# fplll/fplll

Measured on AMD Instinct MI355X. Metric: enum nodes/sec (BKZ-60 SVP enumeration, dim-180 q-ary lattice), higher is better.
Workload: dtype f64; 1 GPU; BASELINE configs[2]: beta=60 blocks kappa=0,1,2 of the 180-dim q-ary lattice, one Enumeration::enumerate call per step, radius min(0.99 r,1.1 GH), FastEvaluator(1); pruning=LinearPruningParams(60,30), counting_rule=fplll (after the bound test), summed in 64 bit

## Files before the change

fplll_amd/build.py:

```python
import os
import subprocess
import sys

HERE = os.path.dirname(os.path.abspath(__file__))
ROOT = os.path.dirname(HERE)
CSRC = os.path.join(HERE, "csrc")
LIBDIR = os.path.join(HERE, "lib")

HIP_SOURCES = ["enum_kernel.hip", "enum_walk.hip", "enum_kernel_cvp.hip", "enum_walk_cvp.hip", "enum_walk4.hip", "enum_kernel_list.hip", "enum_walk_list.hip", "enum_kernel_cvp_list.hip", "enum_walk_cvp_list.hip", "enum_deal.hip", "enum_order.hip", "enum_host.hip", "gso_kernel.hip", "gso_sweep2.hip", "lll_kernel.hip", "lll_kernel_early.hip", "hlll_kernel.hip", "hh_blocked.hip", "hh_rows.hip", "hlll_x.hip", "lll_x.hip", "bkz_kernel.hip", "bkzs_kernel.hip", "bkz_kernel_u.hip", "bkzs_kernel_u.hip", "hlll_kernel_u.hip", "hlll_x_u.hip", "lll_x_u.hip", "gso_host.hip", "lll_gram.hip", "gram_host.hip", "cvp_prepare.hip", "list_vectors.hip", "pruner_volume.hip", "pruner_search.hip", "gso_util_host.hip"]
HIP_HEADERS = ["dev_mem.h", "dev_cache.h", "trace.h", "pruner_tables.h", "pruner_engine.h", "enum_device.h", "enum_order.h", "enum_wave.h", "gso_device.h", "gram_device.h", "gso_wave.h", "gso_sweep2.h", "ftx.h", "lll_wave.h", "lll_stream.h", os.path.join(ROOT, "include", "fplll_hip.h")]
HIPCC_FLAGS = [
    "--offload-arch=gfx950", "-O3", "-std=c++17",
    "-ffp-contract=off",
    "-fPIC", "-Wno-unused-value", "-Wno-inline-asm",
]


PER_FILE_FLAGS = {
    "enum_kernel.hip": ["-mllvm", "-structurizecfg-skip-uniform-regions=1", "-Xclang", "-disable-lifetime-markers"],
    "enum_walk.hip": ["-mllvm", "-structurizecfg-skip-uniform-regions=1", "-Xclang", "-disable-lifetime-markers"],
    "enum_kernel_cvp.hip": ["-mllvm", "-structurizecfg-skip-uniform-regions=1", "-Xclang", "-disable-lifetime-markers"],
    "enum_walk_cvp.hip": ["-mllvm", "-structurizecfg-skip-uniform-regions=1", "-Xclang", "-disable-lifetime-markers"],
    "enum_kernel_list.hip": ["-mllvm", "-structurizecfg-skip-uniform-regions=1", "-Xclang", "-disable-lifetime-markers"],
    "enum_walk_list.hip": ["-mllvm", "-structurizecfg-skip-uniform-regions=1", "-Xclang", "-disable-lifetime-markers"],
    "enum_kernel_cvp_list.hip": ["-mllvm", "-structurizecfg-skip-uniform-regions=1", "-Xclang", "-disable-lifetime-markers"],
    "enum_walk_cvp_list.hip": ["-mllvm", "-structurizecfg-skip-uniform-regions=1", "-Xclang", "-disable-lifetime-markers"],
    "enum_walk4.hip": ["-mllvm", "-structurizecfg-skip-uniform-regions=1", "-Xclang", "-disable-lifetime-markers"],
    "bkzs_kernel.hip": ["-mllvm", "-structurizecfg-skip-uniform-regions=1", "-Xclang", "-disable-lifetime-markers"],
    "bkzs_kernel_u.hip": ["-mllvm", "-structurizecfg-skip-uniform-regions=1", "-Xclang", "-disable-lifetime-markers"],
    "bkz_kernel_u.hip": ["-mllvm", "-structurizecfg-skip-uniform-regions=1"],
    "lll_kernel.hip": ["-mllvm", "-structurizecfg-skip-uniform-regions=1"],
    "lll_kernel_early.hip": ["-mllvm", "-structurizecfg-skip-uniform-regions=1"],
    "lll_gram.hip": ["-mllvm", "-structurizecfg-skip-uniform-regions=1"],
    "bkz_kernel.hip": ["-mllvm", "-structurizecfg-skip-uniform-regions=1"],
    "hlll_kernel.hip": ["-mllvm", "-structurizecfg-skip-uniform-regions=1"],
    "hlll_kernel_u.hip": ["-mllvm", "-structurizecfg-skip-uniform-regions=1"],
    "gso_kernel.hip": ["-mllvm", "-structurizecfg-skip-uniform-regions=1"],
}


EXTRA_DEPS = {"lll_kernel_early.hip": ["lll_kernel.hip"], "enum_kernel_cvp.hip": ["enum_kernel.hip"],
              "enum_walk_cvp.hip": ["enum_walk.hip"], "enum_walk4.hip": ["enum_walk.hip"],
              "enum_kernel_list.hip": ["enum_kernel.hip"], "enum_walk_list.hip": ["enum_walk.hip"],
              "enum_kernel_cvp_list.hip": ["enum_kernel.hip"], "enum_walk_cvp_list.hip": ["enum_walk.hip"], "bkz_kernel_u.hip": ["bkz_kernel.hip"],
              "bkzs_kernel_u.hip": ["bkzs_kernel.hip"], "hlll_kernel_u.hip": ["hlll_kernel.hip"],
              "hlll_x_u.hip": ["hlll_x.hip"], "lll_x_u.hip": ["lll_x.hip"]}


def _newer(target, deps):
    if not os.path.exists(target):
        return True
    t = os.path.getmtime(target)
    return any(os.path.exists(d) and os.path.getmtime(d) > t for d in deps)


def _run(cmd, cwd=None):
    print("[build]", " ".join(cmd), flush=True)
    subprocess.check_call(cmd, cwd=cwd)


def hipcc():
    for c in ("hipcc", "/opt/rocm/bin/hipcc"):
        try:
            subprocess.check_output([c, "--version"], stderr=subprocess.STDOUT)
            return c
        except Exception:
            continue
    raise RuntimeError("hipcc not found")


def build_hip(force=False):
    os.makedirs(LIBDIR, exist_ok=True)
    out = os.path.join(LIBDIR, "libfplll_hip.so")
    srcs = [os.path.join(CSRC, s) for s in HIP_SOURCES if os.path.exists(os.path.join(CSRC, s))]
    hdrs = [h if os.path.isabs(h) else os.path.join(CSRC, h) for h in HIP_HEADERS]
    extra = []
    if os.environ.get("FPHIP_GSO_RING"):
        extra.append("-DFPHIP_GSO_RING=" + os.environ["FPHIP_GSO_RING"])
        force = True
    objdir = os.path.join(LIBDIR, "obj")
    os.makedirs(objdir, exist_ok=True)
    objs = []
    relink = force or not os.path.exists(out)
    jobs = []
    for src in srcs:
        obj = os.path.join(objdir, os.path.basename(src) + ".o")
        objs.append(obj)
        more = [os.path.join(CSRC, x) for x in EXTRA_DEPS.get(os.path.basename(src), [])]
        if force or _newer(obj, [src, os.path.abspath(__file__)] + hdrs + more):
            jobs.append([hipcc()] + HIPCC_FLAGS + extra + PER_FILE_FLAGS.get(os.path.basename(src), []) +
                        ["-c", "-o", obj, src])
            relink = True
    if jobs:
        from concurrent.futures import ThreadPoolExecutor
        with ThreadPoolExecutor(max_workers=max(1, min(len(jobs), os.cpu_count() or 1))) as ex:
# ... 62 lines not shown
```

fplll_amd/csrc/enum_host.hip:

```cpp

#include <hip/hip_runtime.h>

#include <algorithm>
#include <chrono>
#include <cmath>
#include <cstdarg>
#include <cstdio>
#include <cstdlib>
#include <cstring>
#include <vector>

#include "../../include/fplll_hip.h"
#include "dev_mem.h"
#include "trace.h"
#include "enum_device.h"
#include "enum_order.h"


namespace fphip
{
template <bool MU_LDS, bool SUBS, bool DUAL>
__global__ void enum_phase_kernel(DevShared *g, HostCtl *h, TaskBuf in, TaskBuf out, int d,
                                  int Lmax, int stop, unsigned task_lo, unsigned task_hi,
                                  const unsigned *idxlist, int launch_idx, int count_nodes,
                                  unsigned budget, const double *xhi_root, double *gstk, int Tsplit,
                                  unsigned *qh, const unsigned *rcnt, unsigned rcap,
                                  unsigned long long bound_init);
template <int NQT, bool SUBS, bool DUAL>
__global__ void enum_top_kernel(DevShared *g, HostCtl *h, TopBuf in, unsigned n_in, TopBuf out_top,
                                int stop, TaskBuf out, double *xhi_root, int d, double maxdist,
                                int count_nodes, int launch_idx, double *gtop);
__global__ void task_key_kernel(TaskBuf in, unsigned n, int d, unsigned long long *keys,
                                const double *xhi_root, const unsigned *slots);
template <bool MU_LDS, bool DUAL, bool CHAIN>
__global__ void enum_walk_kernel(DevShared *g, HostCtl *h, TaskBuf in, TaskBuf out, int d, int Lmax, unsigned task_lo,
                                 unsigned task_hi, const unsigned *idxlist, int launch_idx, int count_nodes,
                                 unsigned budget, const double *xhi_root, double *gstk, int Tsplit, unsigned *qh,
                                 const unsigned *rcnt, unsigned rcap, unsigned long long bound_init);
template <bool MU_LDS, bool DUAL>
__global__ void enum_walk4_kernel(DevShared *g, HostCtl *h, TaskBuf in, TaskBuf out, int d, int Lmax, unsigned task_lo,
                                  unsigned task_hi, const unsigned *idxlist, int launch_idx, int count_nodes,
                                  unsigned budget, const double *xhi_root, double *gstk, int Tsplit, unsigned *qh,
                                  const unsigned *rcnt, unsigned rcap, unsigned long long bound_init);
template <bool MU_LDS, bool SUBS, bool DUAL>
__global__ void enum_phase_cvp_kernel(DevShared *g, HostCtl *h, TaskBuf in, TaskBuf out, int d, int Lmax, int stop,
                                      unsigned task_lo, unsigned task_hi, const unsigned *idxlist, int launch_idx,
                                      int count_nodes, unsigned budget, const double *xhi_root, double *gstk, int Tsplit,
                                      unsigned *qh, const unsigned *rcnt, unsigned rcap, unsigned long long bound_init);
template <bool MU_LDS, bool DUAL, bool CHAIN>
__global__ void enum_walk_cvp_kernel(DevShared *g, HostCtl *h, TaskBuf in, TaskBuf out, int d, int Lmax, unsigned task_lo,
                                     unsigned task_hi, const unsigned *idxlist, int launch_idx, int count_nodes,
                                     unsigned budget, const double *xhi_root, double *gstk, int Tsplit, unsigned *qh,
                                     const unsigned *rcnt, unsigned rcap, unsigned long long bound_init);
template <bool MU_LDS, bool SUBS, bool DUAL>
__global__ void enum_phase_list_kernel(DevShared *g, HostCtl *h, TaskBuf in, TaskBuf out, int d, int Lmax, int stop,
                                       unsigned task_lo, unsigned task_hi, const unsigned *idxlist, int launch_idx,
                                       int count_nodes, unsigned budget, const double *xhi_root, double *gstk, int Tsplit,
                                       unsigned *qh, const unsigned *rcnt, unsigned rcap, unsigned long long bound_init,
                                       ListBuf lst);
template <bool MU_LDS, bool SUBS, bool DUAL>
__global__ void enum_phase_cvp_list_kernel(DevShared *g, HostCtl *h, TaskBuf in, TaskBuf out, int d, int Lmax, int stop,
                                           unsigned task_lo, unsigned task_hi, const unsigned *idxlist, int launch_idx,
                                           int count_nodes, unsigned budget, const double *xhi_root, double *gstk,
                                           int Tsplit, unsigned *qh, const unsigned *rcnt, unsigned rcap,
                                           unsigned long long bound_init, ListBuf lst);
template <bool MU_LDS, bool DUAL, bool CHAIN>
__global__ void enum_walk_list_kernel(DevShared *g, HostCtl *h, TaskBuf in, TaskBuf out, int d, int Lmax, unsigned task_lo,
                                      unsigned task_hi, const unsigned *idxlist, int launch_idx, int count_nodes,
                                      unsigned budget, const double *xhi_root, double *gstk, int Tsplit, unsigned *qh,
                                      const unsigned *rcnt, unsigned rcap, unsigned long long bound_init, ListBuf lst);
template <bool MU_LDS, bool DUAL, bool CHAIN>
__global__ void enum_walk_cvp_list_kernel(DevShared *g, HostCtl *h, TaskBuf in, TaskBuf out, int d, int Lmax,
                                          unsigned task_lo, unsigned task_hi, const unsigned *idxlist, int launch_idx,
                                          int count_nodes, unsigned budget, const double *xhi_root, double *gstk, int Tsplit,
                                          unsigned *qh, const unsigned *rcnt, unsigned rcap, unsigned long long bound_init,
                                          ListBuf lst);
template <bool DUAL>
__global__ void enum_bfs_cvp_kernel(DevShared *g, double maxdist, QueueMem *qm, TaskBuf f0, TaskBuf f1, TaskBuf fin, int L0,
                                    int nlev, int floor_level, float heavy, int count_nodes, int compact_n, int shard_index,
                                    int shard_count);
template <int NQT, bool SUBS, bool DUAL>
__global__ void enum_top_cvp_kernel(DevShared *g, HostCtl *h, TopBuf in, unsigned n_in, TopBuf out_top, int stop,
                                    TaskBuf out, double *xhi_root, int d, double maxdist, int count_nodes, int launch_idx,
                                    double *gtop);
size_t deal_work_bytes(unsigned n);
unsigned deal_tasks_device(hipStream_t s, const unsigned long long *keys, const double *pd, const unsigned *slot_of,
                           unsigned n, unsigned W, unsigned rank, unsigned *mine, void *work, size_t work_bytes);
size_t order_work_bytes(unsigned n);
int order_tasks_device(hipStream_t s, const DevShared *g, TaskBuf in, unsigned n, int d, const unsigned *slots,
                       unsigned *list, void *work, size_t work_bytes, int num_cus, int *sort_passes);
__global__ void task_pack_kernel(TaskBuf in, unsigned lo, unsigned n, double *rec, const double *xhi_root, int xstr);
__global__ void task_unpack_kernel(TaskBuf out, unsigned lo, unsigned n, const double *rec, double *xhi_root, int xstr,
                                   unsigned root_base);
// ... 939 lines not shown
      else if (dual)
        FPHIP_TOP_LAUNCH(2, false, true);
      else if (subs)
        FPHIP_TOP_LAUNCH(2, true, false);
      else
        FPHIP_TOP_LAUNCH(2, false, false);
#undef FPHIP_TOP_LAUNCH
      HIPCHK(ctx, hipGetLastError());
      HIPCHK(ctx, hipEventRecord(ctx->ev[1], ctx->stream));
      uint64_t nsub = 0;
      int rcw       = wait_serving(ctx, d, cb, subcb, user, &nsub);
      if (rcw != FPHIP_OK)
        return rcw;
      float tms = 0;
      HIPCHK(ctx, hipEventElapsedTime(&tms, ctx->ev[0], ctx->ev[1]));
      top_ms += tms;
      ++launch_idx;
      return FPHIP_OK;
    };
    int rct = top_launch(0, 1u, cut, 1u);
    if (rct != FPHIP_OK)
      return rct;
    if (cut > 64)
    {
      unsigned c1 = 0;
      HIPCHK(ctx, hipMemcpy(&c1, ctx->top[1].count, 4, hipMemcpyDeviceToHost));
      if (c1 > cap2)
      {
        snprintf(ctx->err, sizeof ctx->err, "more than %u top tasks: the block stays on the CPU enumerator", cap2);
        return FPHIP_UNSUPPORTED;
      }
      if (c1 > 0)
      {
        const unsigned per_cu = wide ? 4u : (unsigned)std::max<size_t>(1, (160 * 1024) / std::max<size_t>(tlds, 1));
        const unsigned grid   = std::min<unsigned>(c1, (unsigned)ctx->num_cus * std::min(per_cu, wide ? 4u : 8u));
        rct                   = top_launch(1, c1, 64, grid);
        if (rct != FPHIP_OK)
          return rct;
      }
    }
    HIPCHK(ctx, hipMemcpy(&top_tasks, ctx->buf[cur].count, 4, hipMemcpyDeviceToHost));
    if (top_tasks > top_out.cap)
    {
      snprintf(ctx->err, sizeof ctx->err,
               "more than %u surviving nodes at level 64: the block stays on the CPU enumerator", top_out.cap);
      return FPHIP_UNSUPPORTED;
    }
  }

  const int debug     = env_int("FPHIP_DEBUG", 0);
  const bool walk2    = env_int("FPHIP_WALK2", 1) != 0;
  const bool walk3    = env_int("FPHIP_WALK3", 1) != 0;
  const bool walk4    = env_int("FPHIP_WALK4", 1) != 0;
  uint64_t nsol       = 0;
  double kernel_ms    = top_ms, final_ms = 0.0;
  int launches        = 0;
  int L               = d > 64 ? 64 : d;
  unsigned C          = d > 64 ? top_tasks : 1;
  int final_tasks     = 0, final_L = d;
  const int max_split = env_int("FPHIP_MAX_SPLIT_PHASES", 6);
  double est_nodes = 0;
  for (int k = 0; k < d; ++k)
    est_nodes += std::exp(std::min(logN[k], 60.0));
  unsigned budget       = (unsigned)env_int("FPHIP_BUDGET", 1 << 22);
  const int max_rounds  = env_int("FPHIP_MAX_ROUNDS", 24);
  if (debug)
    fprintf(stderr, "[fphip] d=%d est_nodes=%.3e budget=%u\n", d, est_nodes, budget);
  unsigned long long moved_tasks = 0;
  unsigned xhi_used = d > 64 ? top_tasks : 0;
  bool in_final       = false;
  int round           = 0;
  unsigned prevC      = 0;

  bool regioned = false;
  unsigned n_slots = 0;
  bool bfs_sharded = false;
  if (use_bfs && C > 0)
  {
    FPHIP_RANGE("enum: breadth-first stage");
    const int L0        = L;
    const unsigned rcap = ctx->cap / FPHIP_NQ;
    const double want_tasks = o.target_tasks > 0 ? o.target_tasks : env_int("FPHIP_BFS_TASKS", 65536);
    float heavy = (float)std::max((double)env_int("FPHIP_BFS_HEAVY", 1024), est_nodes / want_tasks);
    int Lend = 1;
    for (int Lv = L0 - 1; Lv >= 1; --Lv)
      if (bfs_est0[Lv] <= heavy)
      {
        Lend = Lv;
        break;
      }
    Lend = std::max(Lend, std::min(L0 - 1, env_int("FPHIP_BFS_FLOOR", 4)));
    const int cnt_bfs = (o.shard_index == 0) ? 1 : 0;
    const bool shard_bfs = o.shard_count > 1 && d <= 64 && o.exchange && env_int("FPHIP_BFS_SHARD", 0) != 0;
    int n_single = 0;
    for (int Lv = L0; Lv > Lend; --Lv)
    {
      const double est_parents = (Lv == L0 ? (double)C : std::exp(std::min(logN[Lv] - logN[L0], 40.0)) * C);
      if (est_parents > env_int("FPHIP_BFS_SINGLE_MAX", 256))
        break;
      ++n_single;
    }
    HIPCHK(ctx, hipEventRecord(ctx->ev[0], ctx->stream));
    int Lv = L0, par = 0;
    int compact_n = (int)C;
    auto bfs_launch = [&](int nlev, unsigned grid, unsigned threads)
    {
// ... 252 lines not shown
          if (got >= 2 && g2 >= 1.0)
            grow = g2;
        }
      cuts.push_back(0u);
      double wsz = (double)first;
      while (cuts.back() < C)
      {
        const bool last = first == 0u || cuts.size() > 128u || launch_idx + (int)cuts.size() + 1 >= FPHIP_MAX_LAUNCHES;
        const double nxtcut = last ? (double)C : std::min((double)C, (double)cuts.back() + std::max(1.0, wsz));
        cuts.push_back((unsigned)nxtcut);
        wsz *= grow;
      }
    }
    const int count_nodes = (in_final || o.shard_index == 0) ? 1 : 0;
    HIPCHK(ctx, hipMemsetAsync(ctx->buf[nxt].count, 0, 4, ctx->stream));

    const int nchunk = order_now ? (int)cuts.size() - 1 : chunks;
    for (int ch = 0; ch < nchunk; ++ch)
    {
      unsigned lo = order_now ? cuts[ch] : (unsigned)(((unsigned long long)n_list * ch) / chunks);
      unsigned hi = order_now ? cuts[ch + 1] : (unsigned)(((unsigned long long)n_list * (ch + 1)) / chunks);
      if (hi <= lo && !(in_final && o.exchange))
        continue;
      unsigned mine = hi - lo;
      unsigned grid = std::min<unsigned>((mine + wpb - 1) / wpb,
                                         (unsigned)(ctx->num_cus * blocks_per_cu));
      if (grid == 0)
        grid = 1;
      if (launch_idx >= FPHIP_MAX_LAUNCHES)
        return fail(ctx, "too many launches");
      if (hi > lo)
      {
        FPHIP_RANGE(in_final ? "enum: walk launch" : "enum: split launch");
        HIPCHK(ctx, hipEventRecord(ctx->ev[0], ctx->stream));
        const unsigned bud =
            (in_final && round < max_rounds && (!subs || env_int("FPHIP_SUBS_DONATE", 1) != 0) && !ordered) ? budget : 0u;
#define FPHIP_LAUNCH(M, S, D) FPHIP_LAUNCH_K(enum_phase_kernel, M, S, D)
#define FPHIP_LAUNCH_K(KERNEL, M, S, D)                                                             \
  hipLaunchKernelGGL((KERNEL<M, S, D>), dim3(grid), dim3(wpb * 64), lds, ctx->stream, ctx->g, \
                     ctx->h, ctx->buf[cur], ctx->buf[nxt], d, L, stop, lo, hi, idxl, launch_idx,     \
                     count_nodes, bud, ctx->xhi_root, ctx->gstk, Ts, &ctx->qm->head[launch_idx][0],          \
                     (regioned && !shard_now && !order_now) ? &ctx->qm->fin[0] : (const unsigned *)nullptr, ctx->cap / FPHIP_NQ, \
                     (unsigned long long)__atomic_load_n(&ctx->h->bound_bits, __ATOMIC_ACQUIRE))
#define FPHIP_LAUNCH2_K(M, D, C) FPHIP_LAUNCH2_KK(enum_walk_kernel, M, D, C)
#define FPHIP_LAUNCH2_KK(KERNEL, M, D, C)                                                            \
  hipLaunchKernelGGL((KERNEL<M, D, C>), dim3(grid), dim3(wpb * 64), lds, ctx->stream, ctx->g, \
                     ctx->h, ctx->buf[cur], ctx->buf[nxt], d, L, lo, hi, idxl, launch_idx,           \
                     count_nodes, bud, ctx->xhi_root, ctx->gstk, Ts, &ctx->qm->head[launch_idx][0],  \
                     (regioned && !shard_now && !order_now) ? &ctx->qm->fin[0] : (const unsigned *)nullptr, ctx->cap / FPHIP_NQ, \
                     (unsigned long long)__atomic_load_n(&ctx->h->bound_bits, __ATOMIC_ACQUIRE))
#define FPHIP_LAUNCH2(M, D)                                                                          \
  do                                                                                                 \
  {                                                                                                  \
    if (walk3 && walk4)                                                                              \
      hipLaunchKernelGGL((enum_walk4_kernel<M, D>), dim3(grid), dim3(wpb * 64), lds, ctx->stream, ctx->g, \
                         ctx->h, ctx->buf[cur], ctx->buf[nxt], d, L, lo, hi, idxl, launch_idx,       \
                         count_nodes, bud, ctx->xhi_root, ctx->gstk, Ts, &ctx->qm->head[launch_idx][0], \
                         (regioned && !shard_now && !order_now) ? &ctx->qm->fin[0] : (const unsigned *)nullptr, ctx->cap / FPHIP_NQ, \
                         (unsigned long long)__atomic_load_n(&ctx->h->bound_bits, __ATOMIC_ACQUIRE)); \
    else if (walk3)                                                                                  \
      FPHIP_LAUNCH2_K(M, D, true);                                                                   \
    else                                                                                             \
      FPHIP_LAUNCH2_K(M, D, false);                                                                  \
  } while (0)
#define FPHIP_LAUNCH_LIST(KERNEL, M)                                                                 \
  hipLaunchKernelGGL((KERNEL<M, false, false>), dim3(grid), dim3(wpb * 64), lds, ctx->stream, ctx->g, \
                     ctx->h, ctx->buf[cur], ctx->buf[nxt], d, L, stop, lo, hi, idxl, launch_idx,     \
                     count_nodes, bud, ctx->xhi_root, ctx->gstk, Ts, &ctx->qm->head[launch_idx][0],  \
                     regioned ? &ctx->qm->fin[0] : (const unsigned *)nullptr, ctx->cap / FPHIP_NQ,   \
                     (unsigned long long)dbits(maxdist), *lst)
#define FPHIP_LAUNCH2_LIST(KERNEL, M, C)                                                             \
  hipLaunchKernelGGL((KERNEL<M, false, C>), dim3(grid), dim3(wpb * 64), lds, ctx->stream, ctx->g,    \
                     ctx->h, ctx->buf[cur], ctx->buf[nxt], d, L, lo, hi, idxl, launch_idx,           \
                     count_nodes, bud, ctx->xhi_root, ctx->gstk, Ts, &ctx->qm->head[launch_idx][0],  \
                     regioned ? &ctx->qm->fin[0] : (const unsigned *)nullptr, ctx->cap / FPHIP_NQ,   \
                     (unsigned long long)dbits(maxdist), *lst)
        if (lst)
        {
          if (in_final && walk2)
          {
            if (cvp && mu_lds && walk3)
              FPHIP_LAUNCH2_LIST(enum_walk_cvp_list_kernel, true, true);
            else if (cvp && mu_lds)
              FPHIP_LAUNCH2_LIST(enum_walk_cvp_list_kernel, true, false);
            else if (cvp && walk3)
              FPHIP_LAUNCH2_LIST(enum_walk_cvp_list_kernel, false, true);
            else if (cvp)
              FPHIP_LAUNCH2_LIST(enum_walk_cvp_list_kernel, false, false);
            else if (mu_lds && walk3)
              FPHIP_LAUNCH2_LIST(enum_walk_list_kernel, true, true);
            else if (mu_lds)
              FPHIP_LAUNCH2_LIST(enum_walk_list_kernel, true, false);
            else if (walk3)
              FPHIP_LAUNCH2_LIST(enum_walk_list_kernel, false, true);
            else
              FPHIP_LAUNCH2_LIST(enum_walk_list_kernel, false, false);
          }
          else if (cvp && mu_lds)
            FPHIP_LAUNCH_LIST(enum_phase_cvp_list_kernel, true);
          else if (cvp)
            FPHIP_LAUNCH_LIST(enum_phase_cvp_list_kernel, false);
          else if (mu_lds)
            FPHIP_LAUNCH_LIST(enum_phase_list_kernel, true);
          else
            FPHIP_LAUNCH_LIST(enum_phase_list_kernel, false);
        }
        else if (cvp)
// ... 319 lines not shown
```

fplll_amd/csrc/enum_walk.hip:

```cpp

#include <hip/hip_runtime.h>
#include <stdint.h>

#include "enum_device.h"
#include "enum_wave.h"

#ifndef FPHIP_CVP
#define FPHIP_CVP 0
#endif
#ifndef FPHIP_LIST
#define FPHIP_LIST 0
#endif
#if FPHIP_LIST && FPHIP_CVP
#define FPHIP_WALK_KERNEL enum_walk_cvp_list_kernel
#elif FPHIP_LIST
#define FPHIP_WALK_KERNEL enum_walk_list_kernel
#elif FPHIP_CVP
#define FPHIP_WALK_KERNEL enum_walk_cvp_kernel
#else
#define FPHIP_WALK_KERNEL enum_walk_kernel
#endif
#if FPHIP_LIST
#define FPHIP_LIST_PARAM , ListBuf lst
#define FPHIP_LIST_TYPE , ListBuf
#else
#define FPHIP_LIST_PARAM
#define FPHIP_LIST_TYPE
#endif
#ifndef FPHIP_WALK4
#define FPHIP_WALK4 0
#endif
#if FPHIP_WALK4
#undef FPHIP_WALK_KERNEL
#define FPHIP_WALK_KERNEL enum_walk4_kernel
#define FPHIP_W4_PAIR 1
#else
#define FPHIP_W4_PAIR 0
#endif

namespace fphip
{

#define ST_I(s) ((s)&0x7f)
#define ST_N(s) (((s) >> 8) & 0x7f)
#define ST_MARK 0x7f64
#define ST_IS_SLOW(s) (((s)&0x7fff) == ST_MARK)
#define ST_IW(s) ((int)((unsigned)(s) >> 17))

__device__ __forceinline__ int zig_of(int i, bool down)
{
  const int hh = (i + 1) >> 1;
  const int z  = (i & 1) ? hh : -hh;
  return down ? -z : z;
}

__device__ __forceinline__ v2u r_issue(const double *tab, unsigned off)
{
  v2u q;
  asm volatile("s_load_dwordx2 %0, %1, %2" : "=s"(q) : "s"(tab), "s"(off));
  return q;
}
__device__ __forceinline__ void rp_wait(v2u &q) { asm volatile("s_waitcnt lgkmcnt(0)" : "+s"(q)); }
__device__ __forceinline__ double rp_r2(const v2u &q) { return __hiloint2double((int)q.y, (int)q.x); }

#if FPHIP_WALK4
template <bool MU_LDS, bool DUAL>
#else
template <bool MU_LDS, bool DUAL, bool CHAIN>
#endif
__global__ void __launch_bounds__(FPHIP_MAX_BLOCK) __attribute__((amdgpu_waves_per_eu(8, 8)))
    FPHIP_WALK_KERNEL(DevShared *__restrict__ g, HostCtl *__restrict__ h, TaskBuf in, TaskBuf out,
                     int d, int Lmax, unsigned task_lo, unsigned task_hi,
                     const unsigned *__restrict__ idxlist, int launch_idx, int count_nodes,
                     unsigned budget, const double *__restrict__ xhi_root, double *__restrict__ gstk,
                     int Tsplit, unsigned *__restrict__ qh, const unsigned *__restrict__ rcnt, unsigned rcap,
                     unsigned long long bound_init FPHIP_LIST_PARAM)
{
  constexpr bool CVP = FPHIP_CVP != 0;
#if FPHIP_WALK4
  constexpr bool CHAIN = true;
#endif
  extern __shared__ __attribute__((aligned(16))) double smem[];
  const int lane = threadIdx.x & 63;
  const int wave = __builtin_amdgcn_readfirstlane((int)(threadIdx.x >> 6));
  constexpr unsigned MUROW8 = FPHIP_MUROW * 8u;
  const unsigned lane8 = (unsigned)lane << 3;
  const int triL = (Lmax * (Lmax + 1)) >> 1;
  const double *mu_s;
  const int nw     = (int)(blockDim.x >> 6);
  const int Ts     = min(Tsplit, Lmax + 1);
  const int Tsm1   = Ts - 1;
  const int ldsRow = tri_off(Ts);
  const int ldsWave = ldsRow + FPHIP_STACK_PAD;
  double *stk;
  if constexpr (MU_LDS)
  {
    double *mu_l = smem;
    stk          = smem + triL + wave * ldsWave;
    const int nmu = (Lmax * (Lmax - 1)) >> 1;
    for (int i = threadIdx.x; i < nmu; i += blockDim.x)
      mu_l[i] = g->mu_tri[i];
    mu_s = mu_l;
  }
  else
  {
    mu_s = &g->mu_sq[0][0];
    stk  = smem + wave * ldsWave;
  }
  if constexpr (MU_LDS)
    __syncthreads();
  const __amdgpu_buffer_rsrc_t mu_b = mu_rsrc(&g->mu_sq[0][0], (unsigned)sizeof(g->mu_sq));
  char *stk_top      = (char *)stk + (((unsigned)ldsRow << 3) + lane8);
  double *gst = gstk + (size_t)(blockIdx.x * nw + wave) * (size_t)(triL - ldsRow + 1) - ldsRow;
  const double *rptab = &g->mu_sq[0][64];
  double zz = (lane & 15) == 0 ? 0.0 : (double)zig_of(lane - (lane >> 4), false);
  FPHIP_IN_VGPR(zz);

  unsigned long long mbits =
      rfl_u64(min(bound_init, __hip_atomic_load(&g->bound_bits, __ATOMIC_RELAXED, __HIP_MEMORY_SCOPE_AGENT)));
  double maxdist   = __longlong_as_double((long long)mbits);
  double maxdist_v = maxdist;
  FPHIP_IN_VGPR(maxdist_v);

  double cs = 0.0, x0s = 0.0, pds = 0.0;
  int st = 0;
  unsigned long long cnt = 0;
  unsigned cnt32         = 0;
  unsigned iter          = 0;
  constexpr int RF = 24;
  int left               = RF - 1;

#define FPHIP_REFRESH_BOUND(from_host, bchg)                                                      \
  do                                                                                              \
  {                                                                                               \
    unsigned long long nb_;                                                                       \
    if (from_host)                                                                                \
    {                                                                                             \
      nb_ = load_sys_u64(&h->bound_bits);                                                         \
      if (nb_ < mbits && lane == 0)                                                               \
        atomicMin(&g->bound_bits, nb_);                                                           \
      FPHIP_JOIN();                                                                               \
    }                                                                                             \
    else                                                                                          \
    {                                                                                             \
      nb_ = __hip_atomic_load(&g->bound_bits, __ATOMIC_RELAXED, __HIP_MEMORY_SCOPE_AGENT);        \
    }                                                                                             \
    nb_ = rfl_u64(nb_);                                                                           \
    if (nb_ < mbits)                                                                              \
    {                                                                                             \
      mbits   = nb_;                                                                              \
      maxdist = __longlong_as_double((long long)mbits);                                           \
      maxdist_v = maxdist;                                                                        \
      FPHIP_IN_VGPR(maxdist_v);                                                                   \
      bchg = true;                                                                                \
    }                                                                                             \
  } while (0)

  unsigned q = (unsigned)__builtin_amdgcn_readfirstlane((int)((blockIdx.x * nw + wave) % FPHIP_NQ));
  const unsigned nlist = task_hi - task_lo;
  for (;;)
  {
    unsigned t = 0, cq = 0;
    bool have = false;
    for (;;)
    {
      if (lane == 0)
        t = atomicAdd(&qh[q * FPHIP_QS], 1u);
      t  = (unsigned)__builtin_amdgcn_readfirstlane((int)t);
// ... 200 lines not shown
        P &= ~gone;
        Q &= ~gone;
      }
#endif
      FPHIP_JOIN();
    };

    enum : int { EV_EMIT = 1, EV_DONE = 3, EV_REFRESH = 6, EV_SPECIAL = 7, EV_FAIL = 8, EV_SLOWSTEP = 10 };
    unsigned elo  = (unsigned)donate;
    unsigned erng = 0x7fffffffu;
    bool buffer_full = false;
    bool resume_step = false;
    double par = 0.0, mk = 0.0;
    double xk = 0.0, a = 0.0;
    int kc = 0;
    double mk1 = 0.0, c1 = 0.0, x1 = 0.0, a1 = 0.0;
#define FPHIP_PUSH(in_lds, kk, lds8)                                            \
  if (__builtin_expect(in_lds, 1))                                              \
    *(double *)(stk_top - (lds8)) = S;                                          \
  else                                                                          \
  {                                                                             \
    int kt = (kk);                                                              \
    asm volatile("" : "+s"(kt));                                                \
    const unsigned gk8 = ((unsigned)(kt * (kt - 1)) << 2) + lane8;              \
    *(double *)((char *)gst + ((lane < kt) ? gk8 : (unsigned)triL << 3)) = S;   \
  }
#define FPHIP_LOAD_PAR_MK()                                                     \
  do                                                                            \
  {                                                                             \
    const unsigned k8_  = (unsigned)k << 3;                                     \
    const unsigned cl8_ = min(lane8, k8_ - 8u);                                 \
    if (k + 1 < Ts)                                                             \
      par = *(const double *)(stk_top - tri8(k + 2));                           \
    else                                                                        \
      par = ld_off(gst, tri8(k + 1) + cl8_);                                    \
    if constexpr (MU_LDS)                                                       \
      mk = ld_off(mu_s, tri8(k) + cl8_);                                        \
    else                                                                        \
      mk = ld_row(mu_b, (unsigned)k * MUROW8, lane8);                           \
  } while (0)
    for (;;)
    {
      int ev;
      bool at_step = resume_step;
      resume_step  = false;
      unsigned spec_t = zc ? 0u : (elo >= 2u ? elo - 2u : 0u);
      spec_t          = (unsigned)__builtin_amdgcn_readfirstlane((int)spec_t);
      int ka = lane_addr(k);
      for (;;)
      {
        if (!at_step)
        {
          kc = k - 1;
          for (;;)
          {
            asm volatile("" : "+s"(kc));
            const unsigned kc8 = (unsigned)kc << 3;
            v4i q1             = rp_issue2(rptab, (unsigned)kc * MUROW8);
            if constexpr (MU_LDS)
              mk1 = ld_off(mu_s, tri8(kc) + min(lane8, kc8 - 8u));
            else
              mk1 = ld_row(mu_b, (unsigned)kc * MUROW8, lane8);
            ka -= 4;
            c1 = bp_f64(S, ka);
            x1 = rint(c1);
            a1 = x1 - c1;
            const double aj  = a1 + zz;
            rp_wait(q1);
            const double bnd = rp_p(q1) * maxdist_v;
            const double ndj = nd + aj * aj * rp_r(q1);
            const unsigned long long m = __builtin_amdgcn_ballot_w64(ndj <= bnd);
            if (m == 0ull)
            {
              ev = EV_FAIL;
              FPHIP_EXIT();
              break;
            }
            if ((unsigned)(kc - 1) >= spec_t)
            {
              ev = EV_SPECIAL;
              FPHIP_EXIT();
              break;
            }
            int c = __builtin_popcountll(m);
            asm("" : "+s"(c));
            if (c == 64)
            {
              ev = EV_SPECIAL;
              FPHIP_EXIT();
              break;
            }
            const unsigned long long me = lane_bit(kc);
            if (CHAIN && c == 4)
            {
              B &= ~me;
              cnt32 = add_bit(me, cnt32);
              nd    = row_bcast0_f64(ndj);
              S     = S - (DUAL ? a1 : x1) * mk1;
              --kc;
              continue;
            }
            if (__builtin_amdgcn_ballot_w64(fabs(a1) == 0.5) != 0ull)
            {
              asm volatile("");
              const bool fix = (a1 < 0.0) == (c1 > 0.0);
              x1             = fix ? x1 - (a1 + a1) : x1;
              a1 = __hiloint2double(__double2hiint(a1) ^ (fix ? (int)0x80000000 : 0), __double2loint(a1));
            }
#if FPHIP_W4_PAIR
            if (c == 5)
            {
              const double sd  = __hiloint2double((c1 >= x1) ? 0x3ff00000 : (int)0xbff00000, 0);
              const double x2  = x1 + sd;
              const double a2  = x2 - c1;
              const double nd2 = nd + a2 * a2 * rp_r(q1);
              const double S1  = S - (DUAL ? a1 : x1) * mk1;
              S                = S - (DUAL ? a2 : x2) * mk1;
              FPHIP_PUSH(kc < Ts - 1, kc + 1, tri8(kc + 2));
              P |= me;
              Q |= me;
              B &= ~me;
              x0s = sel_f64(me, x2, x0s);
              pds = sel_f64(me, nd2, pds);
              cnt32 = add_bit(me, cnt32);
              nd    = row_bcast0_f64(ndj);
              S  = S1;
              --kc;
              continue;
            }
            Q &= ~me;
#endif
            FPHIP_PUSH(kc < Ts - 1, kc + 1, tri8(kc + 2));
            if constexpr (CHAIN)
            {
              P |= me;
              B |= me;
            }
            cs    = sel_f64(me, c1, cs);
            x0s   = sel_f64(me, x1, x0s);
            pds   = sel_f64(me, nd, pds);
            st    = wl_i32((c - 3) << 8, kc, st);
            cnt32 = add_bit(me, cnt32);
            nd    = row_bcast0_f64(ndj);
            S     = S - (DUAL ? a1 : x1) * mk1;
            --kc;
          }
          k = kc + 1;
          ka += 4;
          if (ev != EV_FAIL)
            break;
        }
        at_step = false;
        int tk;
        if constexpr (CHAIN)
        {
          if (__builtin_expect(P == 0ull, 0))
          {
            ev = EV_DONE;
            break;
          }
          k  = __builtin_ctzll(P);
          ka = lane_addr(k);
#if FPHIP_W4_PAIR
          if ((Q >> k) & 1ull)
          {
            if (__builtin_expect(--left < 0, 0))
            {
              ev = EV_REFRESH;
              break;
            }
            const unsigned long long me = lane_bit(k);
            P &= ~me;
            B |= me;
            if (__builtin_expect(k < Tsm1, 1))
              S = *(const double *)(stk_top - tri8(k + 2));
            else
            {
              int kt = k;
              asm volatile("" : "+s"(kt));
              S = ld_off(gst, tri8(kt + 1) + min(lane8, ((unsigned)kt << 3) - 8u));
            }
            nd = bp_f64(pds, ka);
            cnt32 = add_bit(me, cnt32);
            continue;
          }
#endif
          tk = rl_i32(st, k) + 1;
        }
        else
        {
          for (;;)
          {
            tk = rl_i32(st, k) + 1;
            if (__builtin_expect((tk & 0x7f) < ((tk >> 8) & 0x7f), 1))
              break;
            ++k;
            ka += 4;
          }
        }
        if (__builtin_expect((tk & 0x7f) >= 64, 0))
        {
// ... 346 lines not shown
```

fplll_amd/csrc/enum_wave.h:

```cpp
#ifndef FPHIP_ENUM_WAVE_H
#define FPHIP_ENUM_WAVE_H

#include <hip/hip_runtime.h>
#include <stdint.h>

#include "enum_device.h"

namespace fphip
{

__device__ __forceinline__ double rl_f64(double v, int lane)
{
  int lo = __builtin_amdgcn_readlane(__double2loint(v), lane);
  int hi = __builtin_amdgcn_readlane(__double2hiint(v), lane);
  return __hiloint2double(hi, lo);
}
__device__ __forceinline__ int rl_i32(int v, int lane) { return __builtin_amdgcn_readlane(v, lane); }
__device__ __forceinline__ int bp_i32(int v, int addr4) { return __builtin_amdgcn_ds_bpermute(addr4, v); }
__device__ __forceinline__ double bp_f64(double v, int addr4)
{
  return __hiloint2double(bp_i32(__double2hiint(v), addr4), bp_i32(__double2loint(v), addr4));
}
__device__ __forceinline__ double row_bcast0_f64(double v)
{
  double r;
  asm("s_nop 1\n\t"
      "v_mov_b64_dpp %0, %1 row_newbcast:0 row_mask:0xf bank_mask:0xf"
      : "=v"(r)
      : "v"(v));
  return r;
}
__device__ __forceinline__ int lane_addr(int level)
{
  int a = level << 2;
  asm("" : "+v"(a));
  return a;
}
__device__ __forceinline__ double ld_off(const double *row, unsigned off8)
{
  return *(const double *)((const char *)row + off8);
}
typedef unsigned v2u __attribute__((ext_vector_type(2)));
__device__ __forceinline__ __amdgpu_buffer_rsrc_t mu_rsrc(const double *tab, unsigned bytes)
{
  return __builtin_amdgcn_make_buffer_rsrc((void *)tab, 0, bytes, 0x00020000);
}
__device__ __forceinline__ double ld_row(__amdgpu_buffer_rsrc_t tab, unsigned rowoff, unsigned lane8)
{
  const v2u v = __builtin_amdgcn_raw_buffer_load_b64(tab, lane8, rowoff, 0);
  return __hiloint2double((int)v.y, (int)v.x);
}
typedef int v4i __attribute__((ext_vector_type(4)));
__device__ __forceinline__ v4i rp_issue(const double *tab, int level)
{
  v4i q;
  asm volatile("s_load_dwordx4 %0, %1, %2" : "=s"(q) : "s"(tab), "s"(level << 4));
  return q;
}
#ifdef FPHIP_RP_PLAIN
__device__ __forceinline__ v4i rp_issue2(const double *tab, unsigned off)
{
  const v4i *p = (const v4i *)((const char *)tab + off);
  v4i q        = *p;
  q.x = __builtin_amdgcn_readfirstlane(q.x);
  q.y = __builtin_amdgcn_readfirstlane(q.y);
  q.z = __builtin_amdgcn_readfirstlane(q.z);
  q.w = __builtin_amdgcn_readfirstlane(q.w);
  return q;
}
__device__ __forceinline__ void rp_wait(v4i &q) { asm volatile("" : "+s"(q)); }
#else
__device__ __forceinline__ v4i rp_issue2(const double *tab, unsigned off)
{
  v4i q;
  asm volatile("s_load_dwordx4 %0, %1, %2" : "=s"(q) : "s"(tab), "s"(off));
  return q;
}
__device__ __forceinline__ void rp_wait(v4i &q) { asm volatile("s_waitcnt lgkmcnt(0)" : "+s"(q)); }
#endif
__device__ __forceinline__ double rp_r(const v4i &q) { return __hiloint2double(q.y, q.x); }
__device__ __forceinline__ double rp_p(const v4i &q) { return __hiloint2double(q.w, q.z); }
extern "C" __device__ int fphip_llvm_writelane(int, int, int) __asm("llvm.amdgcn.writelane.i32");
// ... 122 lines not shown
```

Measured before the change: 28.75 billion nodes/s.

## Add walk5 enumeration kernel with paired-child zigzag lanes and next-level prefetch

Adds a new enum_walk5 kernel variant, built from enum_walk.hip with FPHIP_WALK5, and makes it the default launch path. The variant changes the lane-to-zigzag-offset mapping so each 16-lane row evaluates paired children (x1±1) and can descend through two siblings at once when no rounding ties occur. It also issues the next level's center, mu-row and rp loads ahead of the current level's bookkeeping to hide memory latency. This adds more register pressure and complex tie and state-encoding paths that must stay consistent with the walk4 semantics and fplll node counting.

```diff
diff --git a/fplll_amd/build.py b/fplll_amd/build.py
--- a/fplll_amd/build.py
+++ b/fplll_amd/build.py
@@ -7,7 +7,7 @@
 CSRC = os.path.join(HERE, "csrc")
 LIBDIR = os.path.join(HERE, "lib")
 
-HIP_SOURCES = ["enum_kernel.hip", "enum_walk.hip", "enum_kernel_cvp.hip", "enum_walk_cvp.hip", "enum_walk4.hip", "enum_kernel_list.hip", "enum_walk_list.hip", "enum_kernel_cvp_list.hip", "enum_walk_cvp_list.hip", "enum_deal.hip", "enum_order.hip", "enum_host.hip", "gso_kernel.hip", "gso_sweep2.hip", "lll_kernel.hip", "lll_kernel_early.hip", "hlll_kernel.hip", "hh_blocked.hip", "hh_rows.hip", "hlll_x.hip", "lll_x.hip", "bkz_kernel.hip", "bkzs_kernel.hip", "bkz_kernel_u.hip", "bkzs_kernel_u.hip", "hlll_kernel_u.hip", "hlll_x_u.hip", "lll_x_u.hip", "gso_host.hip", "lll_gram.hip", "gram_host.hip", "cvp_prepare.hip", "list_vectors.hip", "pruner_volume.hip", "pruner_search.hip", "gso_util_host.hip"]
+HIP_SOURCES = ["enum_kernel.hip", "enum_walk.hip", "enum_kernel_cvp.hip", "enum_walk_cvp.hip", "enum_walk4.hip", "enum_walk5.hip", "enum_kernel_list.hip", "enum_walk_list.hip", "enum_kernel_cvp_list.hip", "enum_walk_cvp_list.hip", "enum_deal.hip", "enum_order.hip", "enum_host.hip", "gso_kernel.hip", "gso_sweep2.hip", "lll_kernel.hip", "lll_kernel_early.hip", "hlll_kernel.hip", "hh_blocked.hip", "hh_rows.hip", "hlll_x.hip", "lll_x.hip", "bkz_kernel.hip", "bkzs_kernel.hip", "bkz_kernel_u.hip", "bkzs_kernel_u.hip", "hlll_kernel_u.hip", "hlll_x_u.hip", "lll_x_u.hip", "gso_host.hip", "lll_gram.hip", "gram_host.hip", "cvp_prepare.hip", "list_vectors.hip", "pruner_volume.hip", "pruner_search.hip", "gso_util_host.hip"]
 HIP_HEADERS = ["dev_mem.h", "dev_cache.h", "trace.h", "pruner_tables.h", "pruner_engine.h", "enum_device.h", "enum_order.h", "enum_wave.h", "gso_device.h", "gram_device.h", "gso_wave.h", "gso_sweep2.h", "ftx.h", "lll_wave.h", "lll_stream.h", os.path.join(ROOT, "include", "fplll_hip.h")]
 HIPCC_FLAGS = [
     "--offload-arch=gfx950", "-O3", "-std=c++17",
@@ -26,6 +26,7 @@
     "enum_kernel_cvp_list.hip": ["-mllvm", "-structurizecfg-skip-uniform-regions=1", "-Xclang", "-disable-lifetime-markers"],
     "enum_walk_cvp_list.hip": ["-mllvm", "-structurizecfg-skip-uniform-regions=1", "-Xclang", "-disable-lifetime-markers"],
     "enum_walk4.hip": ["-mllvm", "-structurizecfg-skip-uniform-regions=1", "-Xclang", "-disable-lifetime-markers"],
+    "enum_walk5.hip": ["-mllvm", "-structurizecfg-skip-uniform-regions=1", "-Xclang", "-disable-lifetime-markers"],
     "bkzs_kernel.hip": ["-mllvm", "-structurizecfg-skip-uniform-regions=1", "-Xclang", "-disable-lifetime-markers"],
     "bkzs_kernel_u.hip": ["-mllvm", "-structurizecfg-skip-uniform-regions=1", "-Xclang", "-disable-lifetime-markers"],
     "bkz_kernel_u.hip": ["-mllvm", "-structurizecfg-skip-uniform-regions=1"],
@@ -40,7 +41,7 @@
 
 
 EXTRA_DEPS = {"lll_kernel_early.hip": ["lll_kernel.hip"], "enum_kernel_cvp.hip": ["enum_kernel.hip"],
-              "enum_walk_cvp.hip": ["enum_walk.hip"], "enum_walk4.hip": ["enum_walk.hip"],
+              "enum_walk_cvp.hip": ["enum_walk.hip"], "enum_walk4.hip": ["enum_walk.hip"], "enum_walk5.hip": ["enum_walk.hip"],
               "enum_kernel_list.hip": ["enum_kernel.hip"], "enum_walk_list.hip": ["enum_walk.hip"],
               "enum_kernel_cvp_list.hip": ["enum_kernel.hip"], "enum_walk_cvp_list.hip": ["enum_walk.hip"], "bkz_kernel_u.hip": ["bkz_kernel.hip"],
               "bkzs_kernel_u.hip": ["bkzs_kernel.hip"], "hlll_kernel_u.hip": ["hlll_kernel.hip"],
diff --git a/fplll_amd/csrc/enum_host.hip b/fplll_amd/csrc/enum_host.hip
--- a/fplll_amd/csrc/enum_host.hip
+++ b/fplll_amd/csrc/enum_host.hip
@@ -39,6 +39,11 @@
                                  const unsigned *rcnt, unsigned rcap, unsigned long long bound_init);
 template <bool MU_LDS, bool DUAL>
 __global__ void enum_walk4_kernel(DevShared *g, HostCtl *h, TaskBuf in, TaskBuf out, int d, int Lmax, unsigned task_lo,
+                                  unsigned task_hi, const unsigned *idxlist, int launch_idx, int count_nodes,
+                                  unsigned budget, const double *xhi_root, double *gstk, int Tsplit, unsigned *qh,
+                                  const unsigned *rcnt, unsigned rcap, unsigned long long bound_init);
+template <bool MU_LDS, bool DUAL>
+__global__ void enum_walk5_kernel(DevShared *g, HostCtl *h, TaskBuf in, TaskBuf out, int d, int Lmax, unsigned task_lo,
                                   unsigned task_hi, const unsigned *idxlist, int launch_idx, int count_nodes,
                                   unsigned budget, const double *xhi_root, double *gstk, int Tsplit, unsigned *qh,
                                   const unsigned *rcnt, unsigned rcap, unsigned long long bound_init);
@@ -1084,6 +1089,7 @@
   const bool walk2    = env_int("FPHIP_WALK2", 1) != 0;
   const bool walk3    = env_int("FPHIP_WALK3", 1) != 0;
   const bool walk4    = env_int("FPHIP_WALK4", 1) != 0;
+  const bool walk5    = env_int("FPHIP_WALK5", 1) != 0;
   uint64_t nsol       = 0;
   double kernel_ms    = top_ms, final_ms = 0.0;
   int launches        = 0;
@@ -1442,7 +1448,13 @@
 #define FPHIP_LAUNCH2(M, D)                                                                          \
   do                                                                                                 \
   {                                                                                                  \
-    if (walk3 && walk4)                                                                              \
+    if (walk3 && walk4 && walk5)                                                                     \
+      hipLaunchKernelGGL((enum_walk5_kernel<M, D>), dim3(grid), dim3(wpb * 64), lds, ctx->stream, ctx->g, \
+                         ctx->h, ctx->buf[cur], ctx->buf[nxt], d, L, lo, hi, idxl, launch_idx,       \
+                         count_nodes, bud, ctx->xhi_root, ctx->gstk, Ts, &ctx->qm->head[launch_idx][0], \
+                         (regioned && !shard_now && !order_now) ? &ctx->qm->fin[0] : (const unsigned *)nullptr, ctx->cap / FPHIP_NQ, \
+                         (unsigned long long)__atomic_load_n(&ctx->h->bound_bits, __ATOMIC_ACQUIRE)); \
+    else if (walk3 && walk4)                                                                         \
       hipLaunchKernelGGL((enum_walk4_kernel<M, D>), dim3(grid), dim3(wpb * 64), lds, ctx->stream, ctx->g, \
                          ctx->h, ctx->buf[cur], ctx->buf[nxt], d, L, lo, hi, idxl, launch_idx,       \
                          count_nodes, bud, ctx->xhi_root, ctx->gstk, Ts, &ctx->qm->head[launch_idx][0], \
diff --git a/fplll_amd/csrc/enum_walk.hip b/fplll_amd/csrc/enum_walk.hip
--- a/fplll_amd/csrc/enum_walk.hip
+++ b/fplll_amd/csrc/enum_walk.hip
@@ -27,6 +27,21 @@
 #define FPHIP_LIST_PARAM
 #define FPHIP_LIST_TYPE
 #endif
+#ifndef FPHIP_WALK5
+#define FPHIP_WALK5 0
+#endif
+#if FPHIP_WALK5
+#define FPHIP_WALK4 1
+#ifndef FPHIP_W5_PAIR
+#define FPHIP_W5_PAIR 1
+#endif
+#ifndef FPHIP_W5_AHEAD
+#define FPHIP_W5_AHEAD 1
+#endif
+#else
+#define FPHIP_W5_PAIR 0
+#define FPHIP_W5_AHEAD 0
+#endif
 #ifndef FPHIP_WALK4
 #define FPHIP_WALK4 0
 #endif
@@ -36,6 +51,10 @@
 #define FPHIP_W4_PAIR 1
 #else
 #define FPHIP_W4_PAIR 0
+#endif
+#if FPHIP_WALK5
+#undef FPHIP_WALK_KERNEL
+#define FPHIP_WALK_KERNEL enum_walk5_kernel
 #endif
 
 namespace fphip
@@ -113,7 +132,12 @@
   char *stk_top      = (char *)stk + (((unsigned)ldsRow << 3) + lane8);
   double *gst = gstk + (size_t)(blockIdx.x * nw + wave) * (size_t)(triL - ldsRow + 1) - ldsRow;
   const double *rptab = &g->mu_sq[0][64];
+#if FPHIP_W5_PAIR
+  double zz = (double)zig_of((lane & 15) < 3 ? (lane & 15) : (lane & 15) + 13 * (lane >> 4), false);
+#define FPHIP_ZONCE 0xfff8fff8fff8ffffull
+#else
   double zz = (lane & 15) == 0 ? 0.0 : (double)zig_of(lane - (lane >> 4), false);
+#endif
   FPHIP_IN_VGPR(zz);
 
   unsigned long long mbits =
@@ -420,8 +444,32 @@
         if (!at_step)
         {
           kc = k - 1;
+#if FPHIP_W5_AHEAD
+          v4i q1;
+          int kb = ka;
+#define FPHIP_NEXT_LEVEL()                                           \
+  do                                                                 \
+  {                                                                  \
+    asm volatile("" : "+s"(kc));                                     \
+    kb -= 4;                                                         \
+    asm("" : "+v"(kb));         \
+    c1 = bp_f64(S, kb);                                              \
+    q1 = rp_issue2(rptab, (unsigned)kc * MUROW8);                    \
+    if constexpr (MU_LDS)                                            \
+      mk1 = ld_off(mu_s, tri8(kc) + min(lane8, ((unsigned)kc << 3) - 8u)); \
+    else                                                             \
+      mk1 = ld_row(mu_b, (unsigned)kc * MUROW8, lane8);              \
+  } while (0)
+          FPHIP_NEXT_LEVEL();
+#else
+#define FPHIP_NEXT_LEVEL() \
+  do                       \
+  {                        \
+  } while (0)
+#endif
           for (;;)
           {
+#if !FPHIP_W5_AHEAD
             asm volatile("" : "+s"(kc));
             const unsigned kc8 = (unsigned)kc << 3;
             v4i q1             = rp_issue2(rptab, (unsigned)kc * MUROW8);
@@ -431,6 +479,7 @@
               mk1 = ld_row(mu_b, (unsigned)kc * MUROW8, lane8);
             ka -= 4;
             c1 = bp_f64(S, ka);
+#endif
             x1 = rint(c1);
             a1 = x1 - c1;
             const double aj  = a1 + zz;
@@ -462,13 +511,62 @@
             if (CHAIN && c == 4)
             {
               B &= ~me;
+#if FPHIP_W5_AHEAD
+              S = S - (DUAL ? a1 : x1) * mk1;
+              --kc;
+              FPHIP_NEXT_LEVEL();
+              cnt32 = add_bit(me, cnt32);
+              nd    = row_bcast0_f64(ndj);
+#else
               cnt32 = add_bit(me, cnt32);
               nd    = row_bcast0_f64(ndj);
               S     = S - (DUAL ? a1 : x1) * mk1;
               --kc;
+#endif
               continue;
             }
+#if FPHIP_W5_PAIR
+            unsigned long long tie = __builtin_amdgcn_ballot_w64(fabs(a1) == 0.5);
+            asm("" : "+s"(tie));
+            if (c == 8)
+            {
+              if (tie != 0ull)
+              {
+                FPHIP_EXIT();
+              }
+              else
+              {
+                double x2, nd2;
+                if ((m & 2ull) != 0ull)
+                {
+                  x2  = x1 + 1.0;
+                  nd2 = row_bcast_f64<1>(ndj);
+                }
+                else
+                {
+                  x2  = x1 - 1.0;
+                  nd2 = row_bcast_f64<2>(ndj);
+                }
+                const double S1 = S - (DUAL ? a1 : x1) * mk1;
+                S               = S - (DUAL ? x2 - c1 : x2) * mk1;
+                FPHIP_PUSH(kc < Ts - 1, kc + 1, tri8(kc + 2));
+                P |= me;
+                Q |= me;
+                B &= ~me;
+                x0s   = sel_f64(me, x2, x0s);
+                pds   = sel_f64(me, nd2, pds);
+                cnt32 = add_bit(me, cnt32);
+                S     = S1;
+                --kc;
+                FPHIP_NEXT_LEVEL();
+                nd = row_bcast0_f64(ndj);
+                continue;
+              }
+            }
+            if (tie != 0ull)
+#else
             if (__builtin_amdgcn_ballot_w64(fabs(a1) == 0.5) != 0ull)
+#endif
             {
               asm volatile("");
               const bool fix = (a1 < 0.0) == (c1 > 0.0);
@@ -476,7 +574,7 @@
               a1 = __hiloint2double(__double2hiint(a1) ^ (fix ? (int)0x80000000 : 0), __double2loint(a1));
             }
 #if FPHIP_W4_PAIR
-            if (c == 5)
+            if (c == (FPHIP_W5_PAIR ? 8 : 5))
             {
               const double sd  = __hiloint2double((c1 >= x1) ? 0x3ff00000 : (int)0xbff00000, 0);
               const double x2  = x1 + sd;
@@ -494,6 +592,7 @@
               nd    = row_bcast0_f64(ndj);
               S  = S1;
               --kc;
+              FPHIP_NEXT_LEVEL();
               continue;
             }
             Q &= ~me;
@@ -507,14 +606,24 @@
             cs    = sel_f64(me, c1, cs);
             x0s   = sel_f64(me, x1, x0s);
             pds   = sel_f64(me, nd, pds);
+#if FPHIP_W5_PAIR
+            st    = wl_i32(__builtin_popcountll(m & FPHIP_ZONCE) << 8, kc, st);
+#else
             st    = wl_i32((c - 3) << 8, kc, st);
+#endif
             cnt32 = add_bit(me, cnt32);
             nd    = row_bcast0_f64(ndj);
             S     = S - (DUAL ? a1 : x1) * mk1;
             --kc;
-          }
+            FPHIP_NEXT_LEVEL();
+          }
+#undef FPHIP_NEXT_LEVEL
           k = kc + 1;
+#if FPHIP_W5_AHEAD
+          ka = lane_addr(k);
+#else
           ka += 4;
+#endif
           if (ev != EV_FAIL)
             break;
         }
diff --git a/fplll_amd/csrc/enum_walk5.hip b/fplll_amd/csrc/enum_walk5.hip
--- /dev/null
+++ b/fplll_amd/csrc/enum_walk5.hip
@@ -0,0 +1,2 @@
+#define FPHIP_WALK5 1
+#include "enum_walk.hip"
diff --git a/fplll_amd/csrc/enum_wave.h b/fplll_amd/csrc/enum_wave.h
--- a/fplll_amd/csrc/enum_wave.h
+++ b/fplll_amd/csrc/enum_wave.h
@@ -28,6 +28,23 @@
       "v_mov_b64_dpp %0, %1 row_newbcast:0 row_mask:0xf bank_mask:0xf"
       : "=v"(r)
       : "v"(v));
+  return r;
+}
+template <int N>
+__device__ __forceinline__ double row_bcast_f64(double v)
+{
+  static_assert(N == 1 || N == 2, "row_newbcast:1 / :2");
+  double r;
+  if constexpr (N == 1)
+    asm("s_nop 1\n\t"
+        "v_mov_b64_dpp %0, %1 row_newbcast:1 row_mask:0xf bank_mask:0xf"
+        : "=v"(r)
+        : "v"(v));
+  else
+    asm("s_nop 1\n\t"
+        "v_mov_b64_dpp %0, %1 row_newbcast:2 row_mask:0xf bank_mask:0xf"
+        : "=v"(r)
+        : "v"(v));
   return r;
 }
 __device__ __forceinline__ int lane_addr(int level)
```

Measured after the change: 29.24 billion nodes/s, median of 6. 1.7% higher.
